# ashvardanian/StringWars

Hardware: AMD Instinct MI355X
Metric: GCUPS (DP cell updates/s) batched Levenshtein (higher is better)
Workload: dtype u32; 1 GPU; C2 tokens64: 1000000 ASCII token pairs per GPU, lengths U[32,96], unbounded Levenshtein, tapes prepared and resident in HBM; step=one synchronous call (results visible on return), pairs_per_gpu=1000000, pairs_total=1000000, cells_per_gpu=4273938131, algorithm=auto, offsets=uint32, collective=none, seed=42

## Files before the change

stringwars_amd/csrc/api.hip:

```cpp
#include <atomic>
#include <chrono>
#include <cstdarg>
#include <cstdio>
#include <cstdlib>
#include <cstring>
#include <new>

#include "api.hpp"
#include <algorithm>
#include <mutex>
#include <utility>

namespace swh {

static thread_local char g_error_text[512];
swh_status_t fail(const char **error, swh_status_t status, const char *fmt, ...) {
    va_list args;
    va_start(args, fmt);
    vsnprintf(g_error_text, sizeof g_error_text, fmt, args);
    va_end(args);
    if (error) *error = g_error_text;
    return status;
}
swh_status_t fail_hip(const char **error, const HipFailure &f) {
// ... 690 lines not shown
            scope->size_belief[0].valid = scope->size_belief[1].valid = false;
            return redo_with(spec);
        }
        if (marker == kUtf8StringTooLong && staged_by_string) {
            scope->utf8_strings_rest = 16;
            CallSpec flat = spec;
            flat.flat_staging = true;
            return redo_with(flat);
        }
        return fail(error, swh_invalid_utf8_k, "invalid UTF-8 in an input tape (marker %u: the string's index when staged string by string, else a 4-byte word inside the 1 KiB tile that failed)", marker - 1);
    }

    swh_status_t run_plan_free() {
        const Route route = rc.route;
        const uint32_t longest = rc.longest;
        scope->summary_slot = (scope->async && dev_out) ? 1u : 0u;
        const bool early = !scope->async && dev_out && !scope->profiling && !invalid_dev && early_return_on() && is_plain_device_memory(spec.out, scope->device);
        if (early) scope->summary_host[0].landed = 0;
        if (route == kRouteDirectShort) launch_direct_short_alone(scope, pre);
        else if (route == kRouteShortTiled) {
            const uint32_t mean_x16 = prepared ? (uint32_t)std::min<uint64_t>(lengths.prepared_mean_x16, 0xFFFFFFu) : scope->hint_mean_x16;
            launch_short_tiled(scope, pre.job, off64, mean_x16);
        }
        else if (route == kRouteCrossShort) launch_cross_short(scope, pre.job, off64, sym_bytes);
        else if (route == kRouteAlignShort) launch_align_short(scope, k, longest, rc.align_wide);
        else if (route == kRouteAlignLong) {
            const uint32_t per_item = align_long_queries(scope, spec.a.count, spec.b.count);
            const uint64_t items = ((uint64_t)(spec.b.count + 63) / 64) * ((uint64_t)(spec.a.count + per_item - 1) / per_item);
            const uint64_t ints = (uint64_t)align_long_waves(scope, items, longest, k.affine != 0) * (longest + 8) * 64 * (k.affine ? 2 : 1);
            ensure(scope->boundary, scope->boundary_bytes, ints * sizeof(int32_t));
            k.boundary = (int32_t *)scope->boundary;
            launch_align_long(scope, k, longest);
        }
        else launch_bitparallel_tiled(scope, k, pairs, longest);
        if (invalid_dev) SWH_HIP_CHECK(hipMemcpyAsync(invalid_host, invalid_dev, 4 * (kUtf8AsciiWord + 2), hipMemcpyDeviceToHost, stream));
        copy_results_back();
        scope->summary_sym_bytes = need_sizes ? 0 : sym_bytes;
        scope->summary_pairs = pairs; scope->summary_ow = ow; scope->summary_elem = elem;
        scope->summary_strings = spec.cross ? (uint64_t)spec.a.count + spec.b.count : 2 * (uint64_t)pairs;
        scope->summary_extra_bytes = need_sizes ? a_bytes + b_bytes : 0;
        scope->summary_pending = true;
        scope->stamps_pending = scope->profiling;
        if (scope->async && dev_out) return swh_success_k;
        if (early) wait_for_summary(scope, stream);
        else SWH_HIP_CHECK(hipStreamSynchronize(stream));
        if (*invalid_host) return utf8_flagged();
        learn_ascii();
        if (scope->summary_host[0].max_la >= kStringLimit || scope->summary_host[0].max_lb >= kStringLimit) {
            scope->summary_pending = false;
            scope->stamps_pending = false;
            scope->hint_lengths = false;
            return fail(error, swh_unsupported_length_k, "a string of 2^30 symbols or more (the longest: %u x %u symbols)",
                        scope->summary_host[0].max_la, scope->summary_host[0].max_lb);
        }
        if (scope->summary_host[0].violation) {
            scope->hint_lengths = false;
            const bool compact_route = (route == kRouteAlignShort && rc.align_wide) || route == kRouteAlignLong;
            const bool compact_failed = compact_route && (scope->summary_host[0].violation & 2u) != 0;
            if (compact_failed) {
                scope->align_wide_off.engine = engine->uid;
                scope->align_wide_off.a = spec.pa ? (const void *)spec.pa : (const void *)spec.a.data;
                scope->align_wide_off.b = spec.pb ? (const void *)spec.pb : (const void *)spec.b.data;
            }
            CallSpec again = spec;
            again.force_planned = !(compact_failed && prepared);
            if (route == kRouteAlignShort && !rc.align_wide) again.skip_upto = longest <= 16 ? 16u : (longest <= 32 ? 32u : 64u);
// ... 406 lines not shown
}
swh_status_t swh_unified_free(swh_scope_t, void *pointer) {
    if (pointer) (void)hipHostFree(pointer);
    return swh_success_k;
}
swh_status_t swh_device_alloc(swh_scope_t handle, size_t bytes, void **pointer, const char **error) {
    if (!handle || !pointer) return fail(error, swh_invalid_argument_k, "null argument");
    (void)hipSetDevice(((Scope *)handle)->device);
    hipError_t err = hipMalloc(pointer, bytes ? bytes : 1);
    if (err != hipSuccess) return fail_hip(error, HipFailure{err, "hipMalloc"});
    return swh_success_k;
}
swh_status_t swh_device_free(swh_scope_t, void *pointer) {
    if (pointer) (void)hipFree(pointer);
    return swh_success_k;
}
swh_status_t swh_copy_to_device(swh_scope_t handle, void *dst, const void *src, size_t bytes, const char **error) {
    Scope *scope = (Scope *)handle;
    if (!scope) return fail(error, swh_invalid_argument_k, "null scope");
    hipError_t err = hipMemcpyAsync(dst, src, bytes, hipMemcpyHostToDevice, scope->stream);
    if (err == hipSuccess) err = hipStreamSynchronize(scope->stream);
    if (err != hipSuccess) return fail_hip(error, HipFailure{err, "hipMemcpy H2D"});
    return swh_success_k;
}
swh_status_t swh_copy_to_host(swh_scope_t handle, void *dst, const void *src, size_t bytes, const char **error) {
    Scope *scope = (Scope *)handle;
    if (!scope) return fail(error, swh_invalid_argument_k, "null scope");
    hipError_t err = hipMemcpyAsync(dst, src, bytes, hipMemcpyDeviceToHost, scope->stream);
    if (err == hipSuccess) err = hipStreamSynchronize(scope->stream);
    if (err != hipSuccess) return fail_hip(error, HipFailure{err, "hipMemcpy D2H"});
    return swh_success_k;
}

}

void swh::free_prepared(Prepared *p) {
    if (!p) return;
    (void)hipSetDevice(p->device);
    for (void *buffer : p->owned) (void)hipFree(buffer);
    delete p;
}

swh_status_t swh::prepare_tape(Scope *scope, const HostTape &tape, bool utf8, swh_prepared_t *out, const char **error) {
    if (!scope || !out) return fail(error, swh_invalid_argument_k, "null argument");
    *out = nullptr;
    if (scope->pipelined) return fail(error, swh_invalid_argument_k, "prepare tapes before switching the scope to pipelined mode");
    Prepared *p = new Prepared();
    try {
        SWH_HIP_CHECK(hipSetDevice(scope->device));
        hipStream_t stream = scope->stream;
        p->device = scope->device;
        p->utf8 = utf8;
        p->off64 = (uint32_t)tape.off64;
        const size_t ow = tape.off64 ? 8 : 4;
        const bool dev_data = is_device_pointer(tape.data), dev_off = is_device_pointer(tape.offsets);
        p->total_bytes = tape.count || tape.offsets ? read_offset(tape.offsets, tape.off64, tape.count, dev_off, stream) : 0;
        auto own = [&](size_t bytes) -> void * {
            void *buffer = nullptr;
            SWH_HIP_CHECK(hipMalloc(&buffer, bytes ? bytes : 16));
            p->owned.push_back(buffer);
            return buffer;
        };
        const void *data = tape.data, *offsets = tape.offsets;
        if (!dev_data) {
            void *buffer = own(p->total_bytes + 16);
            if (p->total_bytes) SWH_HIP_CHECK(hipMemcpyAsync(buffer, tape.data, p->total_bytes, hipMemcpyHostToDevice, stream));
// ... 28 lines not shown
            u.in = p->bytes; u.off64 = p->off64; u.total_bytes = p->total_bytes; u.slot = 0;
            u.symbols = (uint32_t *)own((p->total_bytes + 4) * sizeof(uint32_t));
            u.offsets = (uint64_t *)own((tape.count + 1) * sizeof(uint64_t));
            void *scratch = nullptr;
            SWH_HIP_CHECK(hipMalloc(&scratch, utf8_scratch_words(p->total_bytes) * sizeof(uint32_t) + 256));
            u.counts = (uint32_t *)scratch;
            u.invalid = words + 4;
            hipError_t decode_error = hipSuccess;
            try { launch_utf8_decode(scope, u); } catch (const HipFailure &f) { decode_error = f.code; }
            launch_tape_longest(scope, u.offsets, 1, tape.count, words + 1);
            uint32_t host_words[8] = {0};
            SWH_HIP_CHECK(hipMemcpyAsync(host_words, words, sizeof host_words, hipMemcpyDeviceToHost, stream));
            SWH_HIP_CHECK(hipMemcpyAsync(&total_symbols, u.offsets + tape.count, sizeof(uint64_t), hipMemcpyDeviceToHost, stream));
            SWH_HIP_CHECK(hipStreamSynchronize(stream));
            (void)hipFree(scratch);
            if (decode_error != hipSuccess) throw HipFailure{decode_error, "UTF-8 decode"};
            if (host_words[4]) {
                free_prepared(p);
                return fail(error, swh_invalid_utf8_k, "invalid UTF-8 in the tape (marker %u: a 4-byte word inside the 1 KiB tile that failed)", host_words[4] - 1);
            }
            p->longest_bytes = host_words[0];
            p->longest_symbols = host_words[1];
            p->symbols = TapeRef{u.symbols, u.offsets, tape.count};
            p->ascii = total_symbols == p->total_bytes;
        } else {
            uint32_t host_words[2] = {0, 0};
            SWH_HIP_CHECK(hipMemcpyAsync(host_words, words, sizeof host_words, hipMemcpyDeviceToHost, stream));
            SWH_HIP_CHECK(hipStreamSynchronize(stream));
            p->longest_bytes = p->longest_symbols = host_words[0];
            p->symbols = p->bytes;
        }
        p->total_symbols = total_symbols;
        p->first_byte = std::min(first_byte, p->total_bytes);
        *out = (swh_prepared_t)p;
        return swh_success_k;
    } catch (const HipFailure &f) {
        free_prepared(p);
        return fail_hip(error, f);
    } catch (const std::bad_alloc &) {
        free_prepared(p);
        return fail(error, swh_bad_alloc_k, "host allocation failed");
    }
}

extern "C" {
static swh_status_t upload_matrix(Engine *engine, const int8_t *matrix, const char **error) {
    hipError_t err = hipMalloc((void **)&engine->matrix_dev, 65536);
    if (err == hipSuccess) err = hipMemcpy(engine->matrix_dev, matrix, 65536, hipMemcpyHostToDevice);
    if (err != hipSuccess) return fail_hip(error, HipFailure{err, "substitution matrix upload"});
    engine->scoring.matrix = engine->matrix_dev;
    return swh_success_k;
}

swh_status_t swh_levenshtein_init(swh_scope_t handle, int match, int mismatch, int open, int extend,
                                  swh_levenshtein_t *out, const char **error) {
    if (!handle || !out) return fail(error, swh_invalid_argument_k, "null argument");
    if (match < 0 || mismatch < 0 || open < 0 || extend < 0 || match > 127 || mismatch > 127 || open > 4096 ||
        extend > 4096)
        return fail(error, swh_invalid_argument_k, "Levenshtein costs must be small non-negative integers");
    Scope *scope = (Scope *)handle;
    Engine *engine = new Engine{};
    engine->kind = 0;
    engine->device = scope->device;
    engine->unit_costs = match == 0 && mismatch == 1 && open == 1 && extend == 1;
    engine->algorithm = swh_algorithm_auto_k;
    engine->scoring = Scoring{-match, -mismatch, -open, -extend, nullptr, nullptr};
// ... 208 lines not shown
                                  int32_t *out, size_t stride, const char **error) {
    if (!a || !b) return fail(error, swh_invalid_argument_k, "null tape");
    return nw_pairs(e, 2, s, SWH_TAPE(a, 0), SWH_TAPE(b, 0), out, stride, error);
}
swh_status_t swh_sw_pairs_u64tape(swh_sw_t e, swh_scope_t s, const swh_tape_u64_t *a, const swh_tape_u64_t *b,
                                  int32_t *out, size_t stride, const char **error) {
    if (!a || !b) return fail(error, swh_invalid_argument_k, "null tape");
    return nw_pairs(e, 2, s, SWH_TAPE(a, 1), SWH_TAPE(b, 1), out, stride, error);
}
swh_status_t swh_sw_cross_u64tape(swh_sw_t e, swh_scope_t s, const swh_tape_u64_t *a, const swh_tape_u64_t *b,
                                  ptrdiff_t *out, size_t row_stride, const char **error) {
    return cross_call(e, 2, s, a, b, false, out, row_stride, error);
}

swh_status_t swh_tape_prepare_u32(swh_scope_t scope, const swh_tape_u32_t *tape, int utf8, swh_prepared_t *prepared, const char **error) {
    if (!tape) return fail(error, swh_invalid_argument_k, "null tape");
    return prepare_tape((Scope *)scope, SWH_TAPE(tape, 0), utf8 != 0, prepared, error);
}
swh_status_t swh_tape_prepare_u64(swh_scope_t scope, const swh_tape_u64_t *tape, int utf8, swh_prepared_t *prepared, const char **error) {
    if (!tape) return fail(error, swh_invalid_argument_k, "null tape");
    return prepare_tape((Scope *)scope, SWH_TAPE(tape, 1), utf8 != 0, prepared, error);
}
swh_status_t swh_prepared_info(swh_prepared_t handle, swh_prepared_info_t *info) {
    const Prepared *p = (const Prepared *)handle;
    if (!p || !info) return swh_invalid_argument_k;
    info->count = (size_t)p->bytes.count;
    info->bytes = p->total_bytes;
    info->symbols = p->total_symbols;
    info->longest = p->utf8 ? p->longest_symbols : p->longest_bytes;
    info->utf8 = p->utf8 ? 1 : 0;
    info->ascii = p->ascii ? 1 : 0;
    return swh_success_k;
}
swh_status_t swh_prepared_free(swh_prepared_t handle) {
    free_prepared((Prepared *)handle);
    return swh_success_k;
}

static swh_status_t prepared_call(void *e, int kind, swh_scope_t s, const swh_prepared_view_t *a, const swh_prepared_view_t *b,
                                  bool cross, uint32_t bound, void *out, size_t stride, const char **error) {
    if (!a || !a->tape) return fail(error, swh_invalid_argument_k, "null prepared view");
    if (e && ((Engine *)e)->kind != kind) return fail(error, swh_invalid_argument_k, "engine kind mismatch");
    const swh_prepared_view_t *bb = (b && b->tape) ? b : (cross ? a : nullptr);
    if (!bb) return fail(error, swh_invalid_argument_k, "null prepared view");
    if (!view_fits(a) || !view_fits(bb)) return fail(error, swh_invalid_argument_k, "view exceeds the prepared tape");
    const Prepared *pa = (const Prepared *)a->tape, *pb = (const Prepared *)bb->tape;
    CallSpec spec{};
    spec.a = HostTape{nullptr, nullptr, a->count, 0};
    spec.b = HostTape{nullptr, nullptr, bb->count, 0};
    spec.cross = cross; spec.utf8 = pa->utf8; spec.bound = bound; spec.out = out;
    if (cross) {
        spec.out_stride = 8; spec.out64 = true;
        spec.row_stride = stride ? stride : bb->count * 8;
        if (spec.row_stride < bb->count * 8) return fail(error, swh_invalid_argument_k, "row_stride_bytes too small");
    } else {
        spec.out_stride = stride ? stride : 4; spec.out64 = false;
        if (spec.out_stride < 4) return fail(error, swh_invalid_argument_k, "out_stride_bytes must be >= 4");
    }
    spec.pa = pa; spec.pb = pb; spec.a_first = a->first; spec.b_first = bb->first;
    return run_call((Scope *)s, (Engine *)e, spec, error);
}
swh_status_t swh_levenshtein_pairs_prepared(swh_levenshtein_t e, swh_scope_t s, const swh_prepared_view_t *a, const swh_prepared_view_t *b,
                                            uint32_t bound, uint32_t *out, size_t stride, const char **error) {
    return prepared_call(e, 0, s, a, b, false, bound, out, stride, error);
}
swh_status_t swh_levenshtein_cross_prepared(swh_levenshtein_t e, swh_scope_t s, const swh_prepared_view_t *a, const swh_prepared_view_t *b,
// ... 23 lines not shown
```

stringwars_amd/csrc/api.hpp:

```cpp
#pragma once
#include "common.hpp"

namespace swh {

__attribute__((format(printf, 3, 4))) swh_status_t fail(const char **error, swh_status_t status, const char *fmt, ...);
swh_status_t fail_hip(const char **error, const HipFailure &f);

void collect_timing(Scope *scope);
void add_to_totals(swh_timing_totals_t &totals, const swh_timing_t &call);
void harvest_timing(Scope *scope, bool complete);

inline size_t pad(size_t n) { return (n + 255) & ~(size_t)255; }
struct Carver {
    char *base; size_t used, cap;
    template <typename T> T *take(size_t n) {
        char *p = base ? base + used : nullptr;
        used += pad(n * sizeof(T));
        return (T *)p;
    }
};
void ensure(char *&buf, size_t &cap, size_t need);
bool is_device_pointer(const void *p);
struct AlignScratch { char *buf = nullptr; size_t bytes = 0; };
AlignScratch *call_scratch(const Scope *scope);

struct HostTape { const uint8_t *data; const void *offsets; size_t count; int off64; };
#define SWH_TAPE(t, w) HostTape{(t)->data, (const void *)(t)->offsets, (t)->count, (w)}

struct Prepared {
    int device = 0;
    bool utf8 = false;
    bool ascii = false;
    uint32_t off64 = 0;
    TapeRef bytes{};
    TapeRef symbols{};
    uint64_t total_bytes = 0, total_symbols = 0;
    uint64_t first_byte = 0;
    uint32_t longest_bytes = 0, longest_symbols = 0;
    std::vector<void *> owned;
};
swh_status_t prepare_tape(Scope *scope, const HostTape &tape, bool utf8, swh_prepared_t *out, const char **error);
void free_prepared(Prepared *p);

struct CallSpec {
    HostTape a, b;
    bool cross, utf8;
    uint32_t bound;
    void *out; size_t out_stride, row_stride; bool out64;
    const Prepared *pa = nullptr, *pb = nullptr;
    size_t a_first = 0, b_first = 0;
    bool force_planned = false;
    uint32_t skip_upto = 0;
    bool flat_staging = false;
};
swh_status_t run_call_on(Scope *scope, const Engine *engine, const CallSpec &spec, const char **error);

bool view_fits(const swh_prepared_view_t *view);
swh_status_t check_prepared_pair(const Scope *scope, const Prepared *pa, const Prepared *pb, const char **error);
TapeRef prepared_view(const Prepared *p, bool code_points, size_t first, size_t count);
uint64_t read_offset(const void *offs, int off64, size_t i, bool device, hipStream_t stream);

enum Route { kRoutePlanned, kRouteTiled, kRouteDirectShort, kRouteShortTiled, kRouteCrossShort, kRouteAlignShort, kRouteAlignLong };
struct Lengths {
    bool known = false, guaranteed = false;
    uint32_t la_max = 0, lb_max = 0;
    uint64_t prepared_mean_x16 = 0;
};
Lengths call_lengths(const Scope *scope, const Engine *engine, const CallSpec &spec, bool utf8);
struct RouteChoice {
    Route route = kRoutePlanned;
    uint32_t longest = 0;
    bool align_wide = false;
};
// ... 4 lines not shown
```

stringwars_amd/csrc/tiled.hip:

```cpp
#include <cstdio>
#include <cstdlib>

#include "bp_item.hpp"

namespace swh {

constexpr int tile_index_bits(int waves) { return waves >= 16 ? 12 : 11; }
constexpr int tile_max(int waves) { return 1 << tile_index_bits(waves); }
constexpr uint32_t kAffixCap = 16;
constexpr int kTileBuckets = 32;
constexpr int kTileClasses = 64;
constexpr int kTileBins = kTileClasses * kTileBuckets;

template <int kTileMax>
struct TileLds {
    uint32_t sorted[kTileMax];
    uint32_t bins[kTileBins / 2 > kTileMax / 2 ? kTileBins / 2 : kTileMax / 2];
    uint32_t class_count[kTileClasses];
    uint16_t class_thr[kTileClasses];
    uint16_t class_tgt[kTileClasses];
    uint32_t item_prefix[kTileClasses + 1];
    union {
        uint32_t wave_sums[16];
        struct { unsigned long long lo_a, hi_a, lo_b, hi_b; } span;
    };
    uint32_t ticket;
};
static_assert(sizeof(TileLds<4096>::span) <= sizeof(TileLds<4096>::wave_sums), "the tile's span borrows the scan's wave sums");

__host__ __device__ constexpr uint32_t lane_over(uint32_t x, uint32_t floor_magic) { return (x * floor_magic + x) >> 16; }
constexpr bool lane_over_is_exact() {
    for (uint32_t g = 1; g <= 64; ++g)
        for (uint32_t x = 0; x <= 64; ++x)
            if (lane_over(x, 65535u / g) != x / g) return false;
    return true;
}
static_assert(lane_over_is_exact(), "lane / G and 64 / G by multiplication");

struct TileTail {
    unsigned long long cells, syms;
    uint32_t maxa, maxb, shorts, misfit;
    SummaryLds summary;
};
static_assert(sizeof(TileTail) <= sizeof(uint32_t) * kTileBins / 2, "the tail reuses TileLds::bins");

template <typename Sym, int kWaves> constexpr size_t tiled_lds_bytes() {
    return (size_t)kWaves * (bp_table_words<Sym>() + 64) * 4 + sizeof(TileLds<tile_max(kWaves)>);
}

#ifdef SWH_TILE_PROFILE
__device__ unsigned long long g_tile_phase[8];
__device__ unsigned long long g_tile_span[2048][4];
extern "C" void swh_debug_tile_spans(unsigned long long *out) {
    (void)hipDeviceSynchronize();
    (void)hipMemcpyFromSymbol(out, HIP_SYMBOL(g_tile_span), sizeof(unsigned long long) * 2048 * 4);
}
extern "C" void swh_debug_tile_phases(unsigned long long *out) {
    unsigned long long zero[8] = {};
    (void)hipDeviceSynchronize();
    (void)hipMemcpyFromSymbol(out, HIP_SYMBOL(g_tile_phase), sizeof(zero));
    (void)hipMemcpyToSymbol(HIP_SYMBOL(g_tile_phase), zero, sizeof(zero));
}
#define TILE_STAMP(slot) do { const unsigned long long now__ = __builtin_readcyclecounter(); phase_acc[slot] += now__ - phase_t; phase_t = now__; } while (0)
#else
#define TILE_STAMP(slot) do {} while (0)
#endif

struct TiledArgs {
    KernelArgs k;
    uint32_t tile;
    uint32_t tiles;
    uint32_t shift;
    uint32_t cut_affixes;
    uint32_t no_interior;
    PlanPartial *partials;
    uint32_t *done_counter;
    CallSummary *summary;
};

template <typename Sym, int kWaves, bool kWide, bool kPlain = false>
__device__ __forceinline__ void tiled_run(const TiledArgs &targs, char *smem, const uint64_t a_total, const uint64_t b_total) {
    constexpr int kThreads = kWaves * 64, kTableWords = bp_table_words<Sym>();
    constexpr int kTileMax = tile_max(kWaves), kTileIndexBits = tile_index_bits(kWaves);
    constexpr int kPer = (kTileMax + kThreads - 1) / kThreads;
    constexpr bool kInteriorTiles = sizeof(Sym) == 1 && kWide && kWaves >= 8;
    [[maybe_unused]] KernelArgs shaped;
    const KernelArgs *shaped_or_sent = &targs.k;
    if constexpr (kPlain) {
        shaped = targs.k;
        shaped.off64 = 0; shaped.job.cross = 0; shaped.job.bound = 0xFFFFFFFFu;
        shaped_or_sent = &shaped;
    }
    const KernelArgs &args = *shaped_or_sent;
    const int lane = threadIdx.x & 63, wave = threadIdx.x >> 6;
    BpWave<Sym> wv;
    wv.init((uint32_t *)smem + (size_t)wave * kTableWords, (uint32_t *)smem + (size_t)kWaves * kTableWords + wave * 64, lane,
            a_total, b_total);
    TileLds<kTileMax> &tl = *(TileLds<kTileMax> *)(smem + (size_t)kWaves * (kTableWords + 64) * 4);
    unsigned long long cells = 0, syms = 0;
    uint32_t maxa = 0, maxb = 0, shorts = 0, misfit = 0;
#ifdef SWH_TILE_PROFILE
    unsigned long long phase_acc[4] = {0, 0, 0, 0}, phase_t = __builtin_readcyclecounter(), items_done = 0;
    if (threadIdx.x == 0) g_tile_span[blockIdx.x][0] = __builtin_amdgcn_s_memrealtime();
#endif

    for (uint32_t tile = blockIdx.x; tile < targs.tiles; tile += gridDim.x) {
        const uint64_t base = (uint64_t)tile * targs.tile;
        const uint32_t count = (uint32_t)(args.job.pairs - base < targs.tile ? args.job.pairs - base : targs.tile);
        __builtin_amdgcn_s_setprio(3);
        for (int i = threadIdx.x; i < kTileBins / 2; i += kThreads) tl.bins[i] = 0;
        if (threadIdx.x < kTileClasses) tl.class_count[threadIdx.x] = 0;
        if (threadIdx.x == 0) { tl.ticket = 0; tl.span.lo_a = tl.span.lo_b = ~0ull; tl.span.hi_a = tl.span.hi_b = 0; }
        __syncthreads();
        uint32_t cls[kPer], txt[kPer], rank[kPer], affix[kPer];
        [[maybe_unused]] unsigned long long lo_a = ~0ull, hi_a = 0, lo_b = ~0ull, hi_b = 0;
#ifndef SWH_TILE_BATCH
#define SWH_TILE_BATCH 2
#endif
        constexpr int kBatch = kPer < SWH_TILE_BATCH ? kPer : SWH_TILE_BATCH;
        static_assert(kPer % kBatch == 0, "pairs per thread come in whole batches");
#pragma unroll
        for (int kb = 0; kb < kPer; kb += kBatch) {
        uint64_t a0s[kBatch], b0s[kBatch];
        uint32_t las[kBatch], lbs[kBatch];
#pragma unroll
        for (int j = 0; j < kBatch; ++j) {
            const int k = kb + j;
            const uint64_t p = base + (uint32_t)k * kThreads + threadIdx.x;
            const uint64_t pc = p < args.job.pairs ? p : args.job.pairs - 1;
            if (args.off64) pair_extent<uint64_t, true>(args.job, pc, a0s[j], las[j], b0s[j], lbs[j]);
            else pair_extent<uint32_t, true>(args.job, pc, a0s[j], las[j], b0s[j], lbs[j]);
            affix[k] = 0;
        }
        if constexpr (sizeof(Sym) == 1 && kWide) {
            if (targs.cut_affixes) {
                uint4 ha[kBatch], hb[kBatch], ta[kBatch], tb[kBatch];
                bool inside[kBatch];
#pragma unroll
                for (int j = 0; j < kBatch; ++j) {
                    const uint64_t ea = a0s[j] + las[j], eb = b0s[j] + lbs[j];
                    inside[j] = a0s[j] + 16 <= a_total && b0s[j] + 16 <= b_total && ea >= 16 && eb >= 16;
                    const uint8_t *ad = (const uint8_t *)args.job.a.data, *bd = (const uint8_t *)args.job.b.data;
                    __builtin_memcpy(&ha[j], ad + (inside[j] ? a0s[j] : 0), 16);
                    __builtin_memcpy(&hb[j], bd + (inside[j] ? b0s[j] : 0), 16);
                    __builtin_memcpy(&ta[j], ad + (inside[j] ? ea - 16 : 0), 16);
                    __builtin_memcpy(&tb[j], bd + (inside[j] ? eb - 16 : 0), 16);
                }
#pragma unroll
                for (int j = 0; j < kBatch; ++j) {
                    const uint32_t mn = las[j] < lbs[j] ? las[j] : lbs[j];
                    const unsigned long long h_lo = (unsigned long long)(ha[j].x ^ hb[j].x) | ((unsigned long long)(ha[j].y ^ hb[j].y) << 32);
                    const unsigned long long h_hi = (unsigned long long)(ha[j].z ^ hb[j].z) | ((unsigned long long)(ha[j].w ^ hb[j].w) << 32);
                    const unsigned long long t_lo = (unsigned long long)(ta[j].x ^ tb[j].x) | ((unsigned long long)(ta[j].y ^ tb[j].y) << 32);
                    const unsigned long long t_hi = (unsigned long long)(ta[j].z ^ tb[j].z) | ((unsigned long long)(ta[j].w ^ tb[j].w) << 32);
                    uint32_t pre = h_lo ? (uint32_t)__builtin_ctzll(h_lo) >> 3 : (h_hi ? 8u + ((uint32_t)__builtin_ctzll(h_hi) >> 3) : kAffixCap);
                    pre = pre < mn ? pre : mn;
                    uint32_t suf = t_hi ? (uint32_t)__builtin_clzll(t_hi) >> 3 : (t_lo ? 8u + ((uint32_t)__builtin_clzll(t_lo) >> 3) : kAffixCap);
                    suf = suf < mn - pre ? suf : mn - pre;
                    affix[kb + j] = inside[j] ? pre | (suf << 6) : 0u;
                }
            }
        }
#pragma unroll
        for (int j = 0; j < kBatch; ++j) {
            const int k = kb + j;
            const uint32_t idx = (uint32_t)k * kThreads + threadIdx.x;
            cls[k] = 0xFFu; txt[k] = 0; rank[k] = 0;
            if (idx < count) {
                const uint64_t p = base + idx;
                uint32_t la = las[j], lb = lbs[j];
                if constexpr (kInteriorTiles) {
                    lo_a = a0s[j] < lo_a ? a0s[j] : lo_a; hi_a = a0s[j] + la > hi_a ? a0s[j] + la : hi_a;
                    lo_b = b0s[j] < lo_b ? b0s[j] : lo_b; hi_b = b0s[j] + lb > hi_b ? b0s[j] + lb : hi_b;
                }
                cells += (unsigned long long)la * lb;
                syms += (unsigned long long)la + lb;
                maxa = la > maxa ? la : maxa;
                maxb = lb > maxb ? lb : maxb;
                shorts += (la <= 32 && lb <= 32) ? 1u : 0u;
                if ((la | lb) >= kStringLimit) { misfit = 1; continue; }
                const uint32_t diff = la > lb ? la - lb : lb - la;
                const uint32_t shared = (affix[k] & 63u) + (affix[k] >> 6);
                la -= shared; lb -= shared;
                if (la == 0 || lb == 0) {
                    store_result(args.job, p, (int64_t)clamp_bound(la + lb, args.job.bound));
                } else if (args.job.bound != 0xFFFFFFFFu && diff > args.job.bound) {
                    store_result(args.job, p, (int64_t)args.job.bound + 1);
                } else {
                    const bool pattern_is_a = bp_pattern_is_a(la, lb);
                    const uint32_t m = pattern_is_a ? la : lb, n = pattern_is_a ? lb : la;
                    const uint32_t g = (m + 31) >> 5;
                    if (g > (uint32_t)kTileClasses) {
                        misfit = 1;
                    } else {
                        cls[k] = g - 1;
                        txt[k] = n;
                        affix[k] |= pattern_is_a ? 1u << 12 : 0u;
                        rank[k] = atomicAdd(&tl.class_count[g - 1], 1u);
                    }
                }
            }
        }
        }
        if constexpr (kInteriorTiles) {
            if (!args.off64) {
                lo_a = (uint32_t)~wave_max_u32(~(uint32_t)lo_a); hi_a = wave_max_u32((uint32_t)hi_a);
                lo_b = (uint32_t)~wave_max_u32(~(uint32_t)lo_b); hi_b = wave_max_u32((uint32_t)hi_b);
            } else {
#pragma unroll
                for (int off = 32; off >= 1; off >>= 1) {
                    const unsigned long long la_ = __shfl_xor(lo_a, off), ha_ = __shfl_xor(hi_a, off), lb_ = __shfl_xor(lo_b, off), hb_ = __shfl_xor(hi_b, off);
                    lo_a = la_ < lo_a ? la_ : lo_a; hi_a = ha_ > hi_a ? ha_ : hi_a;
                    lo_b = lb_ < lo_b ? lb_ : lo_b; hi_b = hb_ > hi_b ? hb_ : hi_b;
                }
            }
            if (lane == 0) {
                atomicMin(&tl.span.lo_a, lo_a); atomicMax(&tl.span.hi_a, hi_a);
                atomicMin(&tl.span.lo_b, lo_b); atomicMax(&tl.span.hi_b, hi_b);
            }
        }
        __syncthreads();
        [[maybe_unused]] bool interior = false;
        [[maybe_unused]] BpTileItem ti;
        if constexpr (kInteriorTiles) {
            const unsigned long long s_lo_a = tl.span.lo_a, s_hi_a = tl.span.hi_a, s_lo_b = tl.span.lo_b, s_hi_b = tl.span.hi_b;
            const bool inside = !targs.no_interior && s_lo_a <= s_hi_a && s_lo_b <= s_hi_b && s_lo_a >= kBpMarginLo && s_lo_b >= kBpMarginLo &&
                                s_hi_a <= a_total && s_hi_b <= b_total && a_total - s_hi_a >= kBpMarginHi && b_total - s_hi_b >= kBpMarginHi;
            const unsigned long long da = (unsigned long long)(uintptr_t)args.job.a.data, db = (unsigned long long)(uintptr_t)args.job.b.data;
            const unsigned long long low = (da + s_lo_a < db + s_lo_b ? da + s_lo_a : db + s_lo_b) - kBpMarginLo;
            const unsigned long long top = (da + s_hi_a > db + s_hi_b ? da + s_hi_a : db + s_hi_b) + kBpMarginHi;
            interior = __builtin_amdgcn_readfirstlane((int)(inside && top - low <= (1ull << 31))) != 0;
            if (interior) {
                const uint32_t base_lo = (uint32_t)__builtin_amdgcn_readfirstlane((int)(uint32_t)low), base_hi = (uint32_t)__builtin_amdgcn_readfirstlane((int)(uint32_t)(low >> 32));
                ti.base = (bp_global_bytes)(uintptr_t)(((unsigned long long)base_hi << 32) | base_lo);
                ti.a_off = (uint32_t)__builtin_amdgcn_readfirstlane((int)(uint32_t)(da - low));
                ti.b_off = (uint32_t)__builtin_amdgcn_readfirstlane((int)(uint32_t)(db - low));
                ti.a_last = (uint32_t)__builtin_amdgcn_readfirstlane((int)(uint32_t)(da + s_hi_a + kBpMarginHi - 16 - low));
                ti.b_last = (uint32_t)__builtin_amdgcn_readfirstlane((int)(uint32_t)(db + s_hi_b + kBpMarginHi - 16 - low));
            }
        }
        if (wave == 0) {
            const uint32_t mine = tl.class_count[lane];
            tl.class_thr[lane] = (uint16_t)mine;
            tl.class_tgt[lane] = (uint16_t)lane;
            unsigned long long present = __ballot(mine != 0);
            wave_lds_fence();
            if (lane == 0) {
                uint32_t incoming = 0;
                while (present) {
                    const int c = __builtin_ctzll(present);
                    present &= present - 1;
// ... 39 lines not shown
        {
            constexpr int kWords = (kTileBins / 2 + kThreads - 1) / kThreads;
            uint32_t words[kWords], sum = 0;
#pragma unroll
            for (int q = 0; q < kWords; ++q) {
                const int at = threadIdx.x * kWords + q;
                words[q] = at < kTileBins / 2 ? tl.bins[at] : 0u;
                sum += (words[q] & 0xFFFFu) + (words[q] >> 16);
            }
            const uint32_t incl = wave_inclusive_sum_u32(sum);
            if (lane == 63) tl.wave_sums[wave] = incl;
            __syncthreads();
            uint32_t run = incl - sum;
            for (int w = 0; w < wave; ++w) run += tl.wave_sums[w];
#pragma unroll
            for (int q = 0; q < kWords; ++q) {
                const uint32_t lo = words[q] & 0xFFFFu, hi = words[q] >> 16;
                const int at = threadIdx.x * kWords + q;
                if (at < kTileBins / 2) tl.bins[at] = run | ((run + lo) << 16);
                run += lo + hi;
            }
        }
        __syncthreads();
#pragma unroll
        for (int k = 0; k < kPer; ++k) {
            if (key[k] != 0xFFFFFFFFu) {
                const uint32_t word = tl.bins[key[k] >> 1];
                const uint32_t start = (key[k] & 1u) ? word >> 16 : word & 0xFFFFu;
                tl.sorted[start + rank[k]] = ((uint32_t)k * kThreads + threadIdx.x) | (affix[k] << kTileIndexBits);
            }
        }
        __syncthreads();
        TILE_STAMP(0);
#ifdef SWH_TILE_PROFILE
        if (threadIdx.x == 0) g_tile_span[blockIdx.x][1] = __builtin_amdgcn_s_memrealtime();
#endif
        if (threadIdx.x < kTileClasses) {
            tl.class_thr[threadIdx.x] = (uint16_t)(tl.bins[(threadIdx.x * kTileBuckets) >> 1] & 0xFFFFu);
            tl.class_tgt[threadIdx.x] = (uint16_t)(65535u / (threadIdx.x + 1u));
        }
        __syncthreads();
        static_assert(sizeof(tl.bins) >= (size_t)kTileMax * 2, "the key counters' space holds a tile's distances as 16-bit slots");
        uint16_t *const staged = (uint16_t *)tl.bins;
        for (int i = threadIdx.x; i < kTileMax / 2; i += kThreads) tl.bins[i] = 0xFFFFFFFFu;
        __syncthreads();
        __builtin_amdgcn_s_setprio(0);
        auto run_items = [&](auto mode_tag) {
            constexpr int kMode = decltype(mode_tag)::value;
            const uint32_t items_total = tl.item_prefix[64];
            const uint32_t my_prefix = tl.item_prefix[lane];
            for (;;) {
                uint32_t t = 0;
                if (lane == 0) t = __hip_atomic_fetch_add(&tl.ticket, 1u, __ATOMIC_RELAXED, __HIP_MEMORY_SCOPE_WORKGROUP);
                t = (uint32_t)__builtin_amdgcn_readfirstlane((int)t);
                if (t >= items_total) break;
                const uint32_t item = items_total - 1 - t;
                const uint32_t G = (uint32_t)__popcll(__ballot(my_prefix <= item));
                const uint32_t over_g = (uint32_t)__builtin_amdgcn_readfirstlane((int)(uint32_t)tl.class_tgt[G - 1]);
                const uint32_t per = lane_over(64, over_g);
                const uint32_t chunk = item - tl.item_prefix[G - 1];
                const uint32_t cstart = tl.class_thr[G - 1], ccount = tl.class_count[G - 1];
                const uint32_t slot = lane_over((uint32_t)lane, over_g);
                const uint32_t pidx = chunk * per + slot;
                const bool have = slot < per && pidx < ccount;
                uint64_t p = 0, a0 = 0, b0 = 0;
                uint32_t la = 0, lb = 0;
                BpTileItem mine = ti;
                mine.slot = slot; mine.blk = (uint32_t)lane - slot * G;
                if (have) {
                    const uint32_t entry = tl.sorted[cstart + pidx];
                    p = base + (entry & (uint32_t)(kTileMax - 1));
                    if (args.off64) pair_extent<uint64_t, true>(args.job, p, a0, la, b0, lb);
                    else pair_extent<uint32_t, true>(args.job, p, a0, la, b0, lb);
                    const uint32_t pre = (entry >> kTileIndexBits) & 63u, both = pre + ((entry >> (kTileIndexBits + 6)) & 63u);
                    a0 += pre; b0 += pre; la -= both; lb -= both;
                    mine.a_is_pattern = (entry >> (kTileIndexBits + 12)) & 1u;
                }
                bp_item<Sym, kWide, kMode>(args, wv, G, have, p, a0, la, b0, lb, staged, base, mine);
#ifdef SWH_TILE_PROFILE
                ++items_done;
#endif
            }
        };
        if constexpr (kInteriorTiles) {
            if (interior) run_items(std::integral_constant<int, kBpInterior>{});
            else run_items(std::integral_constant<int, kBpFromTile>{});
        } else if constexpr (sizeof(Sym) == 1) {
            run_items(std::integral_constant<int, kBpFromTile>{});
        } else {
            run_items(std::integral_constant<int, kBpAlone>{});
        }
        TILE_STAMP(1);
        __syncthreads();
        TILE_STAMP(2);
#ifdef SWH_TILE_PROFILE
        if (threadIdx.x == 0) g_tile_span[blockIdx.x][2] = __builtin_amdgcn_s_memrealtime();
#endif
        for (uint32_t i = threadIdx.x; i < count; i += kThreads) {
            const uint32_t d = staged[i];
            if (d != 0xFFFFu) store_result(args.job, base + i, (int64_t)d);
        }
        __syncthreads();
    }
#ifdef SWH_TILE_PROFILE
    if (threadIdx.x == 0) g_tile_span[blockIdx.x][3] = __builtin_amdgcn_s_memrealtime();
    if (lane == 0) {
        for (int q = 0; q < 3; ++q) atomicAdd(&g_tile_phase[q], phase_acc[q]);
        atomicAdd(&g_tile_phase[3], 1ull);
        atomicAdd(&g_tile_phase[4], items_done);
    }
#endif
    {
        TileTail &tail = *(TileTail *)tl.bins;
        unsigned long long &lcells = tail.cells, &lsyms = tail.syms;
        uint32_t &lmaxa = tail.maxa, &lmaxb = tail.maxb, &lshorts = tail.shorts, &lmisfit = tail.misfit;
        if (threadIdx.x == 0) { lcells = 0; lsyms = 0; lmaxa = 0; lmaxb = 0; lshorts = 0; lmisfit = 0; }
        __syncthreads();
#pragma unroll
        for (int off = 32; off >= 1; off >>= 1) {
            cells += __shfl_xor(cells, off);
            syms += __shfl_xor(syms, off);
            shorts += __shfl_xor(shorts, off);
            misfit |= __shfl_xor(misfit, off);
            const uint32_t oa = __shfl_xor(maxa, off), ob = __shfl_xor(maxb, off);
            maxa = oa > maxa ? oa : maxa;
            maxb = ob > maxb ? ob : maxb;
        }
        if (lane == 0) {
            atomicAdd(&lcells, cells);
            atomicAdd(&lsyms, syms);
            atomicMax(&lmaxa, maxa);
            atomicMax(&lmaxb, maxb);
            atomicAdd(&lshorts, shorts);
            atomicOr(&lmisfit, misfit);
        }
        __syncthreads();
        report_call_summary(PlanPartial{lcells, lsyms, lmaxa, lmaxb, lshorts, lmisfit}, targs.partials, targs.done_counter, targs.summary, tail.summary);
    }
}

template <typename Sym, int kWaves, bool kPlain = false>
__global__ __launch_bounds__(kWaves * 64, BpTraits<Sym>::kMinWavesPerSimd) void k_bitparallel_tiled(TiledArgs targs) {
    extern __shared__ __attribute__((aligned(16))) char smem[];
    const KernelArgs &args = targs.k;
    const uint64_t a_total = tape_total(args.job.a, args.off64);
    const uint64_t b_total = tape_total(args.job.b, args.off64);
    if constexpr (sizeof(Sym) == 1) {
        if (a_total >= 16 && b_total >= 16) tiled_run<Sym, kWaves, true, kPlain>(targs, smem, a_total, b_total);
        else tiled_run<Sym, kWaves, false, kPlain>(targs, smem, a_total, b_total);
    } else {
        tiled_run<Sym, kWaves, false, kPlain>(targs, smem, a_total, b_total);
    }
}

TilePlan plan_tiles(uint64_t pairs, uint32_t slots, uint32_t longest_text, uint32_t kTileMax) {
    TilePlan tp{};
    constexpr uint32_t kTileMin = 256;
    const uint64_t rounds = (pairs + (uint64_t)slots * kTileMax - 1) / ((uint64_t)slots * kTileMax);
    uint64_t tile = (pairs + slots * rounds - 1) / (slots * rounds);
    static const uint32_t forced = [] { const char *e = test_hook("STRINGWARS_AMD_TILE"); return e ? (uint32_t)atoi(e) : 0u; }();
    if (forced) tile = forced;
    if (tile < kTileMin) tile = kTileMin;
    if (tile > (uint64_t)kTileMax) tile = kTileMax;
    tp.tile = (uint32_t)tile;
    tp.tiles = (uint32_t)((pairs + tile - 1) / tile);
    tp.blocks = tp.tiles < slots ? tp.tiles : slots;
    uint32_t shift = 0;
    while (((uint64_t)longest_text >> shift) >= (uint64_t)kTileBuckets) ++shift;
    tp.shift = shift;
    return tp;
}

template <typename Sym, int kWaves>
static void launch_tiled_sym(Scope *scope, const KernelArgs &args, uint64_t pairs, uint32_t longest_text) {
    constexpr size_t lds = tiled_lds_bytes<Sym, kWaves>();
    uint32_t slots = (uint32_t)scope->compute_units * (uint32_t)((160 * 1024) / lds);
    if (slots > (uint32_t)kMaxPartials) slots = kMaxPartials;
    const TilePlan tp = plan_tiles(pairs, slots, longest_text, (uint32_t)tile_max(kWaves));
    TiledArgs t{};
    t.k = args;
    t.k.boundary = nullptr;
    t.tile = tp.tile; t.tiles = tp.tiles; t.shift = tp.shift;
    static const bool no_affix = [] { const char *e = test_hook("STRINGWARS_AMD_AFFIX"); return e && atoi(e) == 0; }();
    t.cut_affixes = sizeof(Sym) == 1 && !no_affix ? 1u : 0u;
    static const bool no_interior = [] { const char *e = test_hook("STRINGWARS_AMD_INTERIOR"); return e && atoi(e) == 0; }();
    t.no_interior = no_interior ? 1u : 0u;
    t.partials = scope->plan_partials;
    t.done_counter = scope->done_counter;
    t.summary = scope->summary_target();
    void (*kernel)(TiledArgs) = k_bitparallel_tiled<Sym, kWaves>;
    if constexpr (sizeof(Sym) == 1 && kWaves == 16) {
        if (!args.off64 && !args.job.cross && args.job.bound == 0xFFFFFFFFu) kernel = k_bitparallel_tiled<Sym, kWaves, true>;
    }
    opt_in_dynamic_lds(scope, (const void *)kernel, lds);
    static const bool debug = test_hook("STRINGWARS_AMD_DEBUG") != nullptr;
    if (debug) {
        int per_cu = 0;
        (void)hipOccupancyMaxActiveBlocksPerMultiprocessor(&per_cu, kernel, kWaves * 64, lds);
        fprintf(stderr, "[swh] tiled: pairs %llu tile %u tiles %u blocks %u shift %u lds %zu -> %d workgroups per CU\n",
                (unsigned long long)pairs, tp.tile, tp.tiles, tp.blocks, tp.shift, lds, per_cu);
    }
    StampGuard guard(scope, sizeof(Sym) == 1 ? "bitparallel_tiled" : "bitparallel_tiled_u32");
    hipLaunchKernelGGL(kernel, dim3(tp.blocks), dim3(kWaves * 64), lds, scope->stream, t);
    SWH_HIP_CHECK(hipGetLastError());
}

void launch_bitparallel_tiled(Scope *scope, const KernelArgs &args, uint64_t pairs, uint32_t longest_text) {
    static const int forced = [] { const char *e = test_hook("STRINGWARS_AMD_TILED_WAVES"); return e ? atoi(e) : 0; }();
    if (args.sym_bytes == 4) {
        if (forced == 4) launch_tiled_sym<uint32_t, BpTraits<uint32_t>::kWaves>(scope, args, pairs, longest_text);
        else if (forced == 8) launch_tiled_sym<uint32_t, 8>(scope, args, pairs, longest_text);
        else launch_tiled_sym<uint32_t, 10>(scope, args, pairs, longest_text);
    }
    else if (forced == 4) launch_tiled_sym<uint8_t, 4>(scope, args, pairs, longest_text);
    else if (forced == 8) launch_tiled_sym<uint8_t, 8>(scope, args, pairs, longest_text);
    else if (forced == 16 || (!forced && !scope->async && pairs >= (uint64_t)scope->compute_units * 2048)) launch_tiled_sym<uint8_t, 16>(scope, args, pairs, longest_text);
    else launch_tiled_sym<uint8_t, 8>(scope, args, pairs, longest_text);
}

}
```

Measured before the change: 31840 GCUPS.

## Precompute per-string head/tail 16-byte windows at tape prepare for tiled kernel

```diff
diff --git a/stringwars_amd/csrc/api.hip b/stringwars_amd/csrc/api.hip
--- a/stringwars_amd/csrc/api.hip
+++ b/stringwars_amd/csrc/api.hip
@@ -746,6 +746,8 @@
             k.boundary = (int32_t *)scope->boundary;
             launch_align_long(scope, k, longest);
         }
+        else if (prepared && !utf8 && !spec.cross && spec.pa->side && spec.pb->side)
+            launch_bitparallel_tiled_side(scope, k, pairs, longest, spec.pa->side + 2 * spec.a_first, spec.pb->side + 2 * spec.b_first);
         else launch_bitparallel_tiled(scope, k, pairs, longest);
         if (invalid_dev) SWH_HIP_CHECK(hipMemcpyAsync(invalid_host, invalid_dev, 4 * (kUtf8AsciiWord + 2), hipMemcpyDeviceToHost, stream));
         copy_results_back();
@@ -1218,6 +1220,31 @@
     return swh_success_k;
 }
 
+}
+
+__global__ __launch_bounds__(256) void k_tape_side(const uint8_t *data, const uint32_t *offsets, uint64_t count, uint64_t total, uint4 *side) {
+    const uint64_t i = (uint64_t)blockIdx.x * 256 + threadIdx.x;
+    if (i >= count) return;
+    const int64_t first[2] = {(int64_t)offsets[i], (int64_t)offsets[i + 1] - 16};
+#pragma unroll
+    for (int w = 0; w < 2; ++w) {
+        uint4 v = make_uint4(0, 0, 0, 0);
+        if (first[w] >= 0 && (uint64_t)first[w] + 16 <= total) {
+            __builtin_memcpy(&v, data + first[w], 16);
+        } else {
+            uint8_t bytes[16];
+            for (int j = 0; j < 16; ++j) {
+                const int64_t at = first[w] + j;
+                bytes[j] = at >= 0 && (uint64_t)at < total ? data[at] : (uint8_t)0;
+            }
+            __builtin_memcpy(&v, bytes, 16);
+        }
+        side[2 * i + w] = v;
+    }
+}
+static int side_hook() {
+    static const int choice = [] { const char *e = test_hook("STRINGWARS_AMD_SIDE"); return e ? (atoi(e) != 0 ? 1 : 0) : -1; }();
+    return choice;
 }
 
 void swh::free_prepared(Prepared *p) {
@@ -1312,6 +1339,22 @@
         }
         p->total_symbols = total_symbols;
         p->first_byte = std::min(first_byte, p->total_bytes);
+        const int side_choice = side_hook();
+        const bool side_fits = (!utf8 || p->ascii) && !p->off64 && tape.count > 0;
+        if (side_fits && side_choice != 0 &&
+            (side_choice == 1 || (p->longest_bytes <= tiled_longest_limit() && tape.count >= (uint64_t)scope->compute_units * 2048))) {
+            void *side = nullptr;
+            if (hipMalloc(&side, tape.count * 2 * sizeof(uint4)) == hipSuccess) {
+                p->owned.push_back(side);
+                hipLaunchKernelGGL(k_tape_side, dim3((uint32_t)((tape.count + 255) / 256)), dim3(256), 0, stream, (const uint8_t *)p->bytes.data,
+                                   (const uint32_t *)p->bytes.offsets, (uint64_t)tape.count, p->total_bytes, (uint4 *)side);
+                SWH_HIP_CHECK(hipGetLastError());
+                SWH_HIP_CHECK(hipStreamSynchronize(stream));
+                p->side = (const uint4 *)side;
+            } else {
+                (void)hipGetLastError();
+            }
+        }
         *out = (swh_prepared_t)p;
         return swh_success_k;
     } catch (const HipFailure &f) {
@@ -1586,6 +1629,15 @@
     info->ascii = p->ascii ? 1 : 0;
     return swh_success_k;
 }
+#ifdef SWH_TEST_HOOKS
+size_t swh_debug_prepared_side(swh_prepared_t handle, void *out, size_t strings) {
+    const Prepared *p = (const Prepared *)handle;
+    if (!p || !p->side || !out) return 0;
+    strings = std::min<size_t>(strings, (size_t)p->bytes.count);
+    if (hipSetDevice(p->device) != hipSuccess || hipMemcpy(out, p->side, strings * 32, hipMemcpyDeviceToHost) != hipSuccess) return 0;
+    return strings;
+}
+#endif
 swh_status_t swh_prepared_free(swh_prepared_t handle) {
     free_prepared((Prepared *)handle);
     return swh_success_k;
diff --git a/stringwars_amd/csrc/api.hpp b/stringwars_amd/csrc/api.hpp
--- a/stringwars_amd/csrc/api.hpp
+++ b/stringwars_amd/csrc/api.hpp
@@ -37,8 +37,10 @@
     uint64_t total_bytes = 0, total_symbols = 0;
     uint64_t first_byte = 0;
     uint32_t longest_bytes = 0, longest_symbols = 0;
+    const uint4 *side = nullptr;
     std::vector<void *> owned;
 };
+void launch_bitparallel_tiled_side(Scope *scope, const KernelArgs &args, uint64_t pairs, uint32_t longest_text, const uint4 *side_a, const uint4 *side_b);
 swh_status_t prepare_tape(Scope *scope, const HostTape &tape, bool utf8, swh_prepared_t *out, const char **error);
 void free_prepared(Prepared *p);
 
diff --git a/stringwars_amd/csrc/tiled.hip b/stringwars_amd/csrc/tiled.hip
--- a/stringwars_amd/csrc/tiled.hip
+++ b/stringwars_amd/csrc/tiled.hip
@@ -1,6 +1,8 @@
+#include <atomic>
 #include <cstdio>
 #include <cstdlib>
 
+#include "api.hpp"
 #include "bp_item.hpp"
 
 namespace swh {
@@ -48,13 +50,18 @@
     return (size_t)kWaves * (bp_table_words<Sym>() + 64) * 4 + sizeof(TileLds<tile_max(kWaves)>);
 }
 
-#ifdef SWH_TILE_PROFILE
-__device__ unsigned long long g_tile_phase[8];
+#if defined(SWH_TILE_PROFILE) || defined(SWH_TILE_SPANS)
 __device__ unsigned long long g_tile_span[2048][4];
 extern "C" void swh_debug_tile_spans(unsigned long long *out) {
     (void)hipDeviceSynchronize();
     (void)hipMemcpyFromSymbol(out, HIP_SYMBOL(g_tile_span), sizeof(unsigned long long) * 2048 * 4);
 }
+#define TILE_SPAN(slot) do { if (threadIdx.x == 0) g_tile_span[blockIdx.x][slot] = __builtin_amdgcn_s_memrealtime(); } while (0)
+#else
+#define TILE_SPAN(slot) do {} while (0)
+#endif
+#ifdef SWH_TILE_PROFILE
+__device__ unsigned long long g_tile_phase[8];
 extern "C" void swh_debug_tile_phases(unsigned long long *out) {
     unsigned long long zero[8] = {};
     (void)hipDeviceSynchronize();
@@ -64,6 +71,11 @@
 #define TILE_STAMP(slot) do { const unsigned long long now__ = __builtin_readcyclecounter(); phase_acc[slot] += now__ - phase_t; phase_t = now__; } while (0)
 #else
 #define TILE_STAMP(slot) do {} while (0)
+#endif
+
+#ifdef SWH_TEST_HOOKS
+static std::atomic<unsigned long long> g_tiled_side_launches{0};
+extern "C" unsigned long long swh_debug_tiled_side_launches() { return g_tiled_side_launches.load(); }
 #endif
 
 struct TiledArgs {
@@ -76,9 +88,10 @@
     PlanPartial *partials;
     uint32_t *done_counter;
     CallSummary *summary;
+    const uint4 *side_a, *side_b;
 };
 
-template <typename Sym, int kWaves, bool kWide, bool kPlain = false>
+template <typename Sym, int kWaves, bool kWide, bool kPlain = false, bool kSide = false>
 __device__ __forceinline__ void tiled_run(const TiledArgs &targs, char *smem, const uint64_t a_total, const uint64_t b_total) {
     constexpr int kThreads = kWaves * 64, kTableWords = bp_table_words<Sym>();
     constexpr int kTileMax = tile_max(kWaves), kTileIndexBits = tile_index_bits(kWaves);
@@ -93,42 +106,70 @@
     }
     const KernelArgs &args = *shaped_or_sent;
     const int lane = threadIdx.x & 63, wave = threadIdx.x >> 6;
+    static_assert(!kSide || (kPlain && kWide && sizeof(Sym) == 1), "side arrays: the headline shape only");
     BpWave<Sym> wv;
-    wv.init((uint32_t *)smem + (size_t)wave * kTableWords, (uint32_t *)smem + (size_t)kWaves * kTableWords + wave * 64, lane,
-            a_total, b_total);
+    const auto init_tables = [&] {
+        wv.init((uint32_t *)smem + (size_t)wave * kTableWords, (uint32_t *)smem + (size_t)kWaves * kTableWords + wave * 64, lane,
+                a_total, b_total);
+    };
+    if constexpr (!kSide) init_tables();
     TileLds<kTileMax> &tl = *(TileLds<kTileMax> *)(smem + (size_t)kWaves * (kTableWords + 64) * 4);
     unsigned long long cells = 0, syms = 0;
     uint32_t maxa = 0, maxb = 0, shorts = 0, misfit = 0;
 #ifdef SWH_TILE_PROFILE
     unsigned long long phase_acc[4] = {0, 0, 0, 0}, phase_t = __builtin_readcyclecounter(), items_done = 0;
-    if (threadIdx.x == 0) g_tile_span[blockIdx.x][0] = __builtin_amdgcn_s_memrealtime();
-#endif
+#endif
+    TILE_SPAN(0);
 
     for (uint32_t tile = blockIdx.x; tile < targs.tiles; tile += gridDim.x) {
         const uint64_t base = (uint64_t)tile * targs.tile;
         const uint32_t count = (uint32_t)(args.job.pairs - base < targs.tile ? args.job.pairs - base : targs.tile);
+#ifndef SWH_TILE_BATCH
+#define SWH_TILE_BATCH 2
+#endif
+        constexpr int kBatch = kPer < SWH_TILE_BATCH ? kPer : SWH_TILE_BATCH;
+        static_assert(kPer % kBatch == 0, "pairs per thread come in whole batches");
+        constexpr int kBatchSide = kSide ? kBatch : 1;
+        [[maybe_unused]] uint32_t side_off[kBatchSide][4];
+        [[maybe_unused]] uint4 side_win[kBatchSide][4];
+        [[maybe_unused]] const auto request_side = [&](int kb) {
+            const uint32_t *oa = (const uint32_t *)args.job.a.offsets + base, *ob = (const uint32_t *)args.job.b.offsets + base;
+            const uint4 *sa = targs.side_a + 2 * base, *sb = targs.side_b + 2 * base;
+#pragma unroll
+            for (int j = 0; j < kBatchSide; ++j) {
+                const uint32_t idx = (uint32_t)(kb + j) * kThreads + threadIdx.x, at = idx < count ? idx : count - 1;
+                const uint32_t *xa = (const uint32_t *)((const char *)oa + at * 4u), *xb = (const uint32_t *)((const char *)ob + at * 4u);
+                const uint4 *wa = (const uint4 *)((const char *)sa + at * 32u), *wb = (const uint4 *)((const char *)sb + at * 32u);
+                side_off[j][0] = xa[0]; side_off[j][1] = xa[1]; side_off[j][2] = xb[0]; side_off[j][3] = xb[1];
+                side_win[j][0] = wa[0]; side_win[j][1] = wa[1]; side_win[j][2] = wb[0]; side_win[j][3] = wb[1];
+            }
+        };
+        if constexpr (kSide) {
+            request_side(0);
+            if (tile == blockIdx.x) init_tables();
+        }
         __builtin_amdgcn_s_setprio(3);
         for (int i = threadIdx.x; i < kTileBins / 2; i += kThreads) tl.bins[i] = 0;
         if (threadIdx.x < kTileClasses) tl.class_count[threadIdx.x] = 0;
         if (threadIdx.x == 0) { tl.ticket = 0; tl.span.lo_a = tl.span.lo_b = ~0ull; tl.span.hi_a = tl.span.hi_b = 0; }
         __syncthreads();
         uint32_t cls[kPer], txt[kPer], rank[kPer], affix[kPer];
-        [[maybe_unused]] unsigned long long lo_a = ~0ull, hi_a = 0, lo_b = ~0ull, hi_b = 0;
-#ifndef SWH_TILE_BATCH
-#define SWH_TILE_BATCH 2
-#endif
-        constexpr int kBatch = kPer < SWH_TILE_BATCH ? kPer : SWH_TILE_BATCH;
-        static_assert(kPer % kBatch == 0, "pairs per thread come in whole batches");
+        using Ext = std::conditional_t<kSide, uint32_t, unsigned long long>;
+        [[maybe_unused]] Ext lo_a = (Ext)~0ull, hi_a = 0, lo_b = (Ext)~0ull, hi_b = 0;
 #pragma unroll
         for (int kb = 0; kb < kPer; kb += kBatch) {
-        uint64_t a0s[kBatch], b0s[kBatch];
+        std::conditional_t<kSide, uint32_t, uint64_t> a0s[kBatch], b0s[kBatch];
         uint32_t las[kBatch], lbs[kBatch];
 #pragma unroll
         for (int j = 0; j < kBatch; ++j) {
             const int k = kb + j;
             const uint64_t p = base + (uint32_t)k * kThreads + threadIdx.x;
             const uint64_t pc = p < args.job.pairs ? p : args.job.pairs - 1;
-            if (args.off64) pair_extent<uint64_t, true>(args.job, pc, a0s[j], las[j], b0s[j], lbs[j]);
+            if constexpr (kSide) {
+                a0s[j] = side_off[j][0]; las[j] = side_off[j][1] - side_off[j][0];
+                b0s[j] = side_off[j][2]; lbs[j] = side_off[j][3] - side_off[j][2];
+            }
+            else if (args.off64) pair_extent<uint64_t, true>(args.job, pc, a0s[j], las[j], b0s[j], lbs[j]);
             else pair_extent<uint32_t, true>(args.job, pc, a0s[j], las[j], b0s[j], lbs[j]);
             affix[k] = 0;
         }
@@ -138,6 +179,11 @@
                 bool inside[kBatch];
 #pragma unroll
                 for (int j = 0; j < kBatch; ++j) {
+                    if constexpr (kSide) {
+                        inside[j] = true;
+                        ha[j] = side_win[j][0]; ta[j] = side_win[j][1]; hb[j] = side_win[j][2]; tb[j] = side_win[j][3];
+                        continue;
+                    }
                     const uint64_t ea = a0s[j] + las[j], eb = b0s[j] + lbs[j];
                     inside[j] = a0s[j] + 16 <= a_total && b0s[j] + 16 <= b_total && ea >= 16 && eb >= 16;
                     const uint8_t *ad = (const uint8_t *)args.job.a.data, *bd = (const uint8_t *)args.job.b.data;
@@ -160,6 +206,9 @@
                     affix[kb + j] = inside[j] ? pre | (suf << 6) : 0u;
                 }
             }
+        }
+        if constexpr (kSide) {
+            if (kb + kBatch < kPer) request_side(kb + kBatch);
         }
 #pragma unroll
         for (int j = 0; j < kBatch; ++j) {
@@ -215,8 +264,8 @@
                 }
             }
             if (lane == 0) {
-                atomicMin(&tl.span.lo_a, lo_a); atomicMax(&tl.span.hi_a, hi_a);
-                atomicMin(&tl.span.lo_b, lo_b); atomicMax(&tl.span.hi_b, hi_b);
+                atomicMin(&tl.span.lo_a, (unsigned long long)lo_a); atomicMax(&tl.span.hi_a, (unsigned long long)hi_a);
+                atomicMin(&tl.span.lo_b, (unsigned long long)lo_b); atomicMax(&tl.span.hi_b, (unsigned long long)hi_b);
             }
         }
         __syncthreads();
@@ -322,9 +371,7 @@
         }
         __syncthreads();
         TILE_STAMP(0);
-#ifdef SWH_TILE_PROFILE
-        if (threadIdx.x == 0) g_tile_span[blockIdx.x][1] = __builtin_amdgcn_s_memrealtime();
-#endif
+        TILE_SPAN(1);
         if (threadIdx.x < kTileClasses) {
             tl.class_thr[threadIdx.x] = (uint16_t)(tl.bins[(threadIdx.x * kTileBuckets) >> 1] & 0xFFFFu);
             tl.class_tgt[threadIdx.x] = (uint16_t)(65535u / (threadIdx.x + 1u));
@@ -383,17 +430,15 @@
         TILE_STAMP(1);
         __syncthreads();
         TILE_STAMP(2);
-#ifdef SWH_TILE_PROFILE
-        if (threadIdx.x == 0) g_tile_span[blockIdx.x][2] = __builtin_amdgcn_s_memrealtime();
-#endif
+        TILE_SPAN(2);
         for (uint32_t i = threadIdx.x; i < count; i += kThreads) {
             const uint32_t d = staged[i];
             if (d != 0xFFFFu) store_result(args.job, base + i, (int64_t)d);
         }
         __syncthreads();
     }
+    TILE_SPAN(3);
 #ifdef SWH_TILE_PROFILE
-    if (threadIdx.x == 0) g_tile_span[blockIdx.x][3] = __builtin_amdgcn_s_memrealtime();
     if (lane == 0) {
         for (int q = 0; q < 3; ++q) atomicAdd(&g_tile_phase[q], phase_acc[q]);
         atomicAdd(&g_tile_phase[3], 1ull);
@@ -441,6 +486,15 @@
     } else {
         tiled_run<Sym, kWaves, false, kPlain>(targs, smem, a_total, b_total);
     }
+}
+
+template <int kWaves>
+__global__ __launch_bounds__(kWaves * 64, BpTraits<uint8_t>::kMinWavesPerSimd) void k_bitparallel_tiled_side(TiledArgs targs) {
+    extern __shared__ __attribute__((aligned(16))) char smem[];
+    const KernelArgs &args = targs.k;
+    const uint64_t a_total = tape_total<uint32_t>(args.job.a), b_total = tape_total<uint32_t>(args.job.b);
+    if (a_total >= 16 && b_total >= 16) tiled_run<uint8_t, kWaves, true, true, true>(targs, smem, a_total, b_total);
+    else tiled_run<uint8_t, kWaves, false, true>(targs, smem, a_total, b_total);
 }
 
 TilePlan plan_tiles(uint64_t pairs, uint32_t slots, uint32_t longest_text, uint32_t kTileMax) {
@@ -462,7 +516,7 @@
 }
 
 template <typename Sym, int kWaves>
-static void launch_tiled_sym(Scope *scope, const KernelArgs &args, uint64_t pairs, uint32_t longest_text) {
+static void launch_tiled_sym(Scope *scope, const KernelArgs &args, uint64_t pairs, uint32_t longest_text, const uint4 *side_a, const uint4 *side_b) {
     constexpr size_t lds = tiled_lds_bytes<Sym, kWaves>();
     uint32_t slots = (uint32_t)scope->compute_units * (uint32_t)((160 * 1024) / lds);
     if (slots > (uint32_t)kMaxPartials) slots = kMaxPartials;
@@ -480,7 +534,16 @@
     t.summary = scope->summary_target();
     void (*kernel)(TiledArgs) = k_bitparallel_tiled<Sym, kWaves>;
     if constexpr (sizeof(Sym) == 1 && kWaves == 16) {
-        if (!args.off64 && !args.job.cross && args.job.bound == 0xFFFFFFFFu) kernel = k_bitparallel_tiled<Sym, kWaves, true>;
+        if (!args.off64 && !args.job.cross && args.job.bound == 0xFFFFFFFFu) {
+            kernel = k_bitparallel_tiled<Sym, kWaves, true>;
+            if (side_a && side_b && t.cut_affixes) {
+                kernel = k_bitparallel_tiled_side<kWaves>;
+                t.side_a = side_a; t.side_b = side_b;
+#ifdef SWH_TEST_HOOKS
+                ++g_tiled_side_launches;
+#endif
+            }
+        }
     }
     opt_in_dynamic_lds(scope, (const void *)kernel, lds);
     static const bool debug = test_hook("STRINGWARS_AMD_DEBUG") != nullptr;
@@ -496,16 +559,20 @@
 }
 
 void launch_bitparallel_tiled(Scope *scope, const KernelArgs &args, uint64_t pairs, uint32_t longest_text) {
+    launch_bitparallel_tiled_side(scope, args, pairs, longest_text, nullptr, nullptr);
+}
+
+void launch_bitparallel_tiled_side(Scope *scope, const KernelArgs &args, uint64_t pairs, uint32_t longest_text, const uint4 *side_a, const uint4 *side_b) {
     static const int forced = [] { const char *e = test_hook("STRINGWARS_AMD_TILED_WAVES"); return e ? atoi(e) : 0; }();
     if (args.sym_bytes == 4) {
-        if (forced == 4) launch_tiled_sym<uint32_t, BpTraits<uint32_t>::kWaves>(scope, args, pairs, longest_text);
-        else if (forced == 8) launch_tiled_sym<uint32_t, 8>(scope, args, pairs, longest_text);
-        else launch_tiled_sym<uint32_t, 10>(scope, args, pairs, longest_text);
-    }
-    else if (forced == 4) launch_tiled_sym<uint8_t, 4>(scope, args, pairs, longest_text);
-    else if (forced == 8) launch_tiled_sym<uint8_t, 8>(scope, args, pairs, longest_text);
-    else if (forced == 16 || (!forced && !scope->async && pairs >= (uint64_t)scope->compute_units * 2048)) launch_tiled_sym<uint8_t, 16>(scope, args, pairs, longest_text);
-    else launch_tiled_sym<uint8_t, 8>(scope, args, pairs, longest_text);
-}
-
-}
+        if (forced == 4) launch_tiled_sym<uint32_t, BpTraits<uint32_t>::kWaves>(scope, args, pairs, longest_text, side_a, side_b);
+        else if (forced == 8) launch_tiled_sym<uint32_t, 8>(scope, args, pairs, longest_text, side_a, side_b);
+        else launch_tiled_sym<uint32_t, 10>(scope, args, pairs, longest_text, side_a, side_b);
+    }
+    else if (forced == 4) launch_tiled_sym<uint8_t, 4>(scope, args, pairs, longest_text, side_a, side_b);
+    else if (forced == 8) launch_tiled_sym<uint8_t, 8>(scope, args, pairs, longest_text, side_a, side_b);
+    else if (forced == 16 || (!forced && !scope->async && pairs >= (uint64_t)scope->compute_units * 2048)) launch_tiled_sym<uint8_t, 16>(scope, args, pairs, longest_text, side_a, side_b);
+    else launch_tiled_sym<uint8_t, 8>(scope, args, pairs, longest_text, side_a, side_b);
+}
+
+}
```

Measured after the change: 34810 GCUPS (median of 6 runs). 9.4% higher.
